# martinambrus/PitchExtractor

Hardware: AMD Instinct MI355X
Metric: mel-frames/sec training throughput (JDCNet, 24 kHz, batch=256) (higher is better)
Workload: dtype f32

## Files before the change

### pitchextractor_amd/csrc/common.h

```cpp
#pragma once
#include <hip/hip_runtime.h>
#include <stdint.h>
#include <stdlib.h>
#include <string.h>
#include "../../include/pitchextractor_hip.h"

#define PE_CHECK_HIP(expr)                              \
  do {                                                  \
    hipError_t _e = (expr);                             \
    if (_e != hipSuccess) return (int)_e;               \
  } while (0)

#define PE_LAUNCH_CHECK()                               \
  do {                                                  \
    hipError_t _e = hipGetLastError();                  \
    if (_e != hipSuccess) return (int)_e;               \
  } while (0)

static inline hipStream_t pe_stream(void* s) { return reinterpret_cast<hipStream_t>(s); }

static inline int pe_unserved(int products) {
  return products >= PE_PROD_NATIVE && products <= PE_PROD_F16 ? PE_E_UNSUPPORTED : PE_E_ARG;
}

static inline int pe_cdiv(long a, long b) { return (int)((a + b - 1) / b); }

static inline int pe_epilogue_buffer(long out_bytes) {
  static const int forced_pointer = [] {
    const char* e = getenv("PE_EPILOGUE");
    return e && strcmp(e, "pointer") == 0 ? 1 : 0;
  }();
  return !forced_pointer && out_bytes < (1L << 31);
}

typedef float f32x4 __attribute__((ext_vector_type(4)));
typedef float f32x16 __attribute__((ext_vector_type(16)));

#define PE_WAVE 64

__device__ __forceinline__ double pe_wave_strided_sum(const double* base, long stride, int n) {
  const int lane = threadIdx.x & 63;
  double s = 0.0;
  for (int z = lane; z < n; z += 64) s += base[(long)z * stride];
#pragma unroll
  for (int off = 32; off > 0; off >>= 1) s += __shfl_down(s, off, 64);
  return s;
}

static inline int pe_pick_splits(int tiles, long K, int min_k_per_split, int resident) {
  long max_s = K / min_k_per_split;
  if (max_s < 1) max_s = 1;
  if (max_s > 1024) max_s = 1024;
  int best = 1;
  double best_score = -1.0;
  for (int sp = 1; sp <= (int)max_s; ++sp) {
    const long wgs = (long)tiles * sp;
    const long waves = (wgs + resident - 1) / resident;
    const double eff = (double)wgs / (double)(waves * resident);
    const double score = eff - 0.0001 * sp + (wgs >= 2L * resident ? 0.05 : 0.0);
    if (score > best_score) { best_score = score; best = sp; }
  }
  return best;
}

__device__ __forceinline__ float4 pe_ordered_slab_sum4(const float* __restrict__ ws, long slab_stride, int splits,
                                                       long i4) {
  const float4* p = reinterpret_cast<const float4*>(ws) + i4;
  const long st4 = slab_stride >> 2;
  double sx = 0.0, sy = 0.0, sz = 0.0, sw = 0.0;
  int z = 0;
  for (; z + 8 <= splits; z += 8) {
    float4 v[8];
#pragma unroll
    for (int u = 0; u < 8; ++u) v[u] = p[(long)(z + u) * st4];
#pragma unroll
    for (int u = 0; u < 8; ++u) { sx += (double)v[u].x; sy += (double)v[u].y; sz += (double)v[u].z; sw += (double)v[u].w; }
  }
  for (; z < splits; ++z) {
    const float4 v = p[(long)z * st4];
    sx += (double)v.x; sy += (double)v.y; sz += (double)v.z; sw += (double)v.w;
  }
  return make_float4((float)sx, (float)sy, (float)sz, (float)sw);
}

__device__ __forceinline__ void philox_round(uint32_t (&c)[4], uint32_t (&k)[2]) {
  const uint32_t M0 = 0xD2511F53u, M1 = 0xCD9E8D57u;
  const uint64_t p0 = (uint64_t)M0 * c[0], p1 = (uint64_t)M1 * c[2];
  const uint32_t n0 = (uint32_t)(p1 >> 32) ^ c[1] ^ k[0];
  const uint32_t n1 = (uint32_t)p1;
  const uint32_t n2 = (uint32_t)(p0 >> 32) ^ c[3] ^ k[1];
  const uint32_t n3 = (uint32_t)p0;
  c[0] = n0; c[1] = n1; c[2] = n2; c[3] = n3;
  k[0] += 0x9E3779B9u; k[1] += 0xBB67AE85u;
}

__device__ __forceinline__ void philox4(uint64_t seed, uint64_t ctr, uint32_t (&out)[4]) {
  uint32_t c[4] = {(uint32_t)ctr, (uint32_t)(ctr >> 32), 0u, 0u};
  uint32_t k[2] = {(uint32_t)seed, (uint32_t)(seed >> 32)};
#pragma unroll
  for (int i = 0; i < 10; ++i) philox_round(c, k);
  out[0] = c[0]; out[1] = c[1]; out[2] = c[2]; out[3] = c[3];
}

__device__ __forceinline__ bool pe_dropout_keep(uint32_t word, float p) {
  return ((float)(word >> 8) * (1.0f / 16777216.0f)) >= p;
}
```

### pitchextractor_amd/csrc/gemm.hip

```cpp
#include <stdlib.h>
#include <type_traits>
#include <utility>
#include "splitk.h"


namespace {
using namespace pe;
typedef unsigned int u32x4 __attribute__((ext_vector_type(4)));

bool aligned16(const void* p) { return (reinterpret_cast<uintptr_t>(p) & 15) == 0; }

template <class TO>
struct StoreEpiT {
  TO* C;
  long ldc;
  const float* bias0;
  const float* bias1;
  int M, N, accumulate;
  __device__ __forceinline__ void operator()(int row, int col, float v) const {
    if (row < M && col < N) {
      if (bias0) v += bias0[col];
      if (bias1) v += bias1[col];
      TO* dst = C + (long)row * ldc + col;
      if (accumulate) v += ld1(dst);
// ... 124 lines not shown
        }
      }
  }
}

template <class TL, class F, class TA = typename F::TA>
int launch_nt(const RowLoaderT<TA>& al, const RowLoader& bl, const StoreEpiT<TA>& ep, int M, int N, int K,
              hipStream_t st, const unsigned* amax_a, const unsigned* amax_b) {
  constexpr int MODE = F::MODE;
  using TH = typename F::TH;
  const int tm = pe_cdiv(M, TL::BM), tn = pe_cdiv(N, TL::BN);
  const bool vec = MODE != kNative && (N & 3) == 0 && (ep.ldc & 3) == 0 &&
                   (reinterpret_cast<uintptr_t>(ep.C) & (4 * sizeof(TA) - 1)) == 0;
  if (vec) {
    if (ep.ldc >= N && pe_epilogue_buffer((long)(M + TL::BM) * ep.ldc * (long)sizeof(TA)))
      hipLaunchKernelGGL((gemm_nt_t_kernel<TL, MODE, true, TA, TH>), dim3(tm * tn), dim3(256), 0, st, al, bl, ep, K, tm,
                         tn, amax_a, amax_b);
    else
      hipLaunchKernelGGL((gemm_nt_t_kernel<TL, MODE, false, TA, TH>), dim3(tm * tn), dim3(256), 0, st, al, bl, ep, K, tm,
                         tn, amax_a, amax_b);
  }
  else
    hipLaunchKernelGGL((gemm_nt_kernel<TL, MODE, TA, TH>), dim3(tm * tn), dim3(256), 0, st, al, bl, ep, K, tm, tn, amax_a,
                       amax_b);
  PE_LAUNCH_CHECK();
  return PE_OK;
}

}

template <class F, class TA = typename F::TA>
static int gemm_nt_impl(const TA* A, long lda, const float* B, long ldb, TA* C, long ldc, int M, int N,
                        int K, const float* bias0, const float* bias1, int accumulate, void* stream,
                        const unsigned* amax_a, const unsigned* amax_b) {
  constexpr int MODE = F::MODE;
  if (!A || !B || !C || M < 0 || N < 0 || K <= 0) return PE_E_ARG;
  if (MODE == kSplit2 && (!amax_a || !amax_b)) return PE_E_ARG;
  if (M == 0 || N == 0) return PE_OK;
  if ((K & 3) || (lda & 3) || (ldb & 3) || (reinterpret_cast<uintptr_t>(A) & (4 * sizeof(TA) - 1)) || !aligned16(B))
    return PE_E_UNSUPPORTED;
  if (lda < 0 || ldb < 0 || lda >= (1L << 21) || ldb >= (1L << 21)) return PE_E_UNSUPPORTED;
  RowLoaderT<TA> al{A, lda, M, K, 0};
  RowLoader bl{B, ldb, N, K, 0};
  StoreEpiT<TA> ep{C, ldc, bias0, bias1, M, N, accumulate};
  hipStream_t st = pe_stream(stream);
  if (N <= 32) return launch_nt<Tile<128, 32, 4, 1>, F>(al, bl, ep, M, N, K, st, amax_a, amax_b);
  if (N <= 64) return launch_nt<Tile<256, 64, 4, 1>, F>(al, bl, ep, M, N, K, st, amax_a, amax_b);
  if (N % 192 == 0 && (N % 128 != 0 || MODE != kNative))
    return launch_nt<Tile<128, 192, 2, 2>, F>(al, bl, ep, M, N, K, st, amax_a, amax_b);
  return launch_nt<Tile<128, 128, 2, 2>, F>(al, bl, ep, M, N, K, st, amax_a, amax_b);
}

extern "C" int pe_gemm_nt(int products, int act16, const void* A, long lda, const float* B, long ldb, void* C, long ldc,
                          int M, int N, int K, const float* bias0, const float* bias1, int accumulate,
                          const unsigned* amax_a, const unsigned* amax_b, void* stream) {
  return with_form<kAllForms, true>(products, act16, [&](auto f) {
    using TA = typename decltype(f)::TA;
    return gemm_nt_impl<decltype(f)>(static_cast<const TA*>(A), lda, B, ldb, static_cast<TA*>(C), ldc, M, N, K, bias0,
                                     bias1, accumulate, stream, amax_a, amax_b);
  });
}

extern "C" size_t pe_gemm_tn_workspace_bytes(int M, int N, int K) {
  if (M <= 0 || N <= 0 || K <= 0) return 0;
  const int s = tn_max_splits(pe_cdiv(M, M <= 64 ? 64 : 128) * pe_cdiv(N, N <= 64 ? 64 : 128), K);
  return s > 1 ? (size_t)s * M * N * sizeof(float) : 0;
}

template <class F, class TA = typename F::TA>
static int gemm_tn_impl(const TA* A, long lda, const TA* B, long ldb, float* C, long ldc, int M, int N,
                        int K, int accumulate, float* workspace, size_t workspace_bytes, void* stream,
                        const unsigned* amax_a, const unsigned* amax_b) {
  constexpr int MODE = F::MODE;
  if (!A || !B || !C || M < 0 || N < 0 || K <= 0) return PE_E_ARG;
  if (MODE == kSplit2 && (!amax_a || !amax_b)) return PE_E_ARG;
  if (M == 0 || N == 0) return PE_OK;
  if ((M & 3) || (N & 3) || (lda & 3) || (ldb & 3) || (reinterpret_cast<uintptr_t>(A) & (4 * sizeof(TA) - 1)) ||
      (reinterpret_cast<uintptr_t>(B) & (4 * sizeof(TA) - 1)))
    return PE_E_UNSUPPORTED;
  if (lda < 0 || ldb < 0 || lda >= (1L << 24) || ldb >= (1L << 24)) return PE_E_UNSUPPORTED;
  hipStream_t st = pe_stream(stream);
  auto launch = [&](auto bm, auto bn) {
    constexpr int BM = decltype(bm)::value, BN = decltype(bn)::value;
    return launch_tn<BM, BN, F>(KRowLoader<BM, TA>{A, lda, M, 0}, KRowLoader<BN, TA>{B, ldb, N, 0}, C, ldc, M, N, K,
                                accumulate, workspace, workspace_bytes, st, amax_a, amax_b);
  };
  std::integral_constant<int, 64> t64;
  std::integral_constant<int, 128> t128;
  if (M <= 64 && N <= 64) return launch(t64, t64);
  if (M <= 64) return launch(t64, t128);
  if (N <= 64) return launch(t128, t64);
  return launch(t128, t128);
}

extern "C" int pe_gemm_tn(int products, int act16, const void* A, long lda, const void* B, long ldb, float* C, long ldc,
                          int M, int N, int K, int accumulate, float* workspace, size_t workspace_bytes,
                          const unsigned* amax_a, const unsigned* amax_b, void* stream) {
  return with_form<kAllForms, true>(products, act16, [&](auto f) {
    using TA = typename decltype(f)::TA;
    return gemm_tn_impl<decltype(f)>(static_cast<const TA*>(A), lda, static_cast<const TA*>(B), ldb, C, ldc, M, N, K,
                                     accumulate, workspace, workspace_bytes, stream, amax_a, amax_b);
  });
}
```

### pitchextractor_amd/csrc/gemm_engine.h

```cpp
#pragma once
#include <type_traits>
#include <utility>
#include "act16.h"

namespace pe {

constexpr int kBK = 32;
constexpr int kNative = 0;
constexpr int kBf16 = 1;
constexpr int kSplit = 2;
constexpr int kSplit2 = 3;
template <int MODE> constexpr int mode_terms() { return MODE == kSplit ? 3 : MODE == kSplit2 ? 2 : 1; }
constexpr int kLdsStride = kBK + 4;

template <int BM_, int BN_, int WAVES_M_, int WAVES_N_>
struct Tile {
  static constexpr int BM = BM_, BN = BN_;
  static constexpr int WAVES_M = WAVES_M_, WAVES_N = WAVES_N_;
  static constexpr int WM = BM / WAVES_M, WN = BN / WAVES_N;
  static constexpr int TM = WM / 32, TN = WN / 32;
  static constexpr int A_LOADS = BM / 32, B_LOADS = BN / 32;
  static_assert(WAVES_M * WAVES_N == 4, "4 waves per workgroup");
  static_assert(WM % 32 == 0 && WN % 32 == 0, "wave tile is a multiple of the 32x32 MFMA");
};
// ... 377 lines not shown
#pragma unroll
      for (int i = 0; i < TL::B_LOADS; ++i) rb[q][i] = bl.load(i, kt + PF);
    }
    if constexpr (PF == 2) __builtin_amdgcn_sched_barrier(0);
#pragma unroll
    for (int kk = 0; kk < kBK / 16; ++kk) {
      half8<H> fa[TL::TM][NT], fb[TL::TN][NT];
#pragma unroll
      for (int i = 0; i < TL::TM; ++i)
#pragma unroll
        for (int c = 0; c < NT; ++c)
          fa[i][c] = *reinterpret_cast<const half8<H>*>(As + c * A_IMG + swz_off(wm * TL::WM + i * 32 + r, kk * 2 + h));
#pragma unroll
      for (int j = 0; j < TL::TN; ++j)
#pragma unroll
        for (int c = 0; c < NT; ++c)
          fb[j][c] = *reinterpret_cast<const half8<H>*>(Bs + c * B_IMG + swz_off(wn * TL::WN + j * 32 + r, kk * 2 + h));
#pragma unroll
      for (int i = 0; i < TL::TM; ++i)
#pragma unroll
        for (int j = 0; j < TL::TN; ++j) acc[i][j] = mfma_terms<NT, SW>(fa[i], fb[j], acc[i][j]);
    }
    if constexpr (PF == 2) __builtin_amdgcn_sched_barrier(0);
  };
  int kt = 0;
  if constexpr (PF == 2) {
    for (; kt + 1 < nk; kt += 2) {
      tile(std::integral_constant<int, 0>{}, kt);
      tile(std::integral_constant<int, 1>{}, kt + 1);
    }
  }
  for (; kt < nk; ++kt) tile(std::integral_constant<int, 0>{}, kt);
}

template <class F, int... Q>
__device__ __forceinline__ void static_for_impl(F&& f, std::integer_sequence<int, Q...>) {
  (f(std::integral_constant<int, Q>{}), ...);
}
template <int N, class F>
__device__ __forceinline__ void static_for(F&& f) { static_for_impl(f, std::make_integer_sequence<int, N>{}); }

template <int MODE> constexpr int nt_row_floats() {
  return MODE == kSplit ? kSplitRowFloats : MODE == kSplit2 ? 2 * kBK / 2 : kLdsStride;
}

template <class TL, int MODE, bool SW = false, int PF = 1, class TH = __bf16, class AL, class BL>
__device__ __forceinline__ void nt_mainloop_mode(AL& al, BL& bl, int K, float* As, float* Bs,
                                                 f32x16 (&acc)[TL::TM][TL::TN], float sa = 1.0f, float sb = 1.0f) {
  if constexpr (MODE == kBf16) nt_mainloop_half<TL, TH>(al, bl, K, As, Bs, acc);
  else if constexpr (MODE == kSplit) nt_mainloop_split<TL, SW, 3, PF>(al, bl, K, As, Bs, acc);
  else if constexpr (MODE == kSplit2) nt_mainloop_split<TL, SW, 2, PF>(al, bl, K, As, Bs, acc, sa, sb);
  else nt_mainloop<TL>(al, bl, K, As, Bs, acc);
}

template <class TL, class FN>
__device__ __forceinline__ void for_each_acc(const f32x16 (&acc)[TL::TM][TL::TN], FN&& fn) {
  const int lane = threadIdx.x & 63, wv = threadIdx.x >> 6;
  const int wm = wv / TL::WAVES_N, wn = wv % TL::WAVES_N;
  const int r = lane & 31, h = lane >> 5;
#pragma unroll
  for (int i = 0; i < TL::TM; ++i)
#pragma unroll
    for (int j = 0; j < TL::TN; ++j)
#pragma unroll
      for (int g = 0; g < 16; ++g) {
        const int row = wm * TL::WM + i * 32 + (g & 3) + 8 * (g >> 2) + 4 * h;
        const int col = wn * TL::WN + j * 32 + r;
        fn(row, col, acc[i][j][g]);
      }
}

template <class TL>
__device__ __forceinline__ void zero_acc(f32x16 (&acc)[TL::TM][TL::TN]) {
#pragma unroll
  for (int i = 0; i < TL::TM; ++i)
#pragma unroll
    for (int j = 0; j < TL::TN; ++j)
#pragma unroll
      for (int g = 0; g < 16; ++g) acc[i][j][g] = 0.0f;
}

template <int COLS>
struct TnGeom {
  static constexpr int TPR = COLS / 4;
  static constexpr int ROWS = 256 / TPR;
  static constexpr int SLOTS = kBK / ROWS;
  static_assert(COLS == 64 || COLS == 128 || COLS == 256, "TN tile widths");
  __device__ static __forceinline__ int col4() { return (threadIdx.x % TPR) * 4; }
  __device__ static __forceinline__ int krow(int slot) { return threadIdx.x / TPR + ROWS * slot; }
};

template <int COLS, class TA = float>
struct KRowLoader {
  const TA* p;
  long ld;
  int cols;
  int col0;
  unsigned vo_ = 0, rowstep_ = 0;
  typedef typename RawQuad<TA>::type Raw;
  __device__ __forceinline__ void init(int first_col, int ) {
    col0 = first_col + TnGeom<COLS>::col4();
    vo_ = (unsigned)(((long)(threadIdx.x / TnGeom<COLS>::TPR) * ld + col0) * (long)sizeof(TA)) | (col0 < cols ? 0u : 0x80000000u);
    rowstep_ = (unsigned)(TnGeom<COLS>::ROWS * ld * (long)sizeof(TA));
  }
  __device__ __forceinline__ Raw load(int slot, int k0, int k_end) const {
    const long left = (long)k_end - k0;
    long bytes = left > 0 ? ((left - 1) * ld + cols) * (long)sizeof(TA) : 0;
    const __amdgpu_buffer_rsrc_t rs = __builtin_amdgcn_make_buffer_rsrc(
        const_cast<TA*>(p + (long)k0 * ld), 0, (unsigned)(bytes < 0x7fffffffL ? bytes : 0x7fffffffL), 0x00020000);
    return ldraw_buffer<TA>(rs, vo_ + (unsigned)slot * rowstep_, 0u);
  }
};

template <int COLS>
struct ShiftedPixelLoader {
  const float* p;
  int T, F, C, dt, df;
  int col0;
  int t_[TnGeom<COLS>::SLOTS], f_[TnGeom<COLS>::SLOTS];
  __device__ __forceinline__ void init(int first_col, int k_begin) {
    col0 = first_col + TnGeom<COLS>::col4();
#pragma unroll
    for (int i = 0; i < TnGeom<COLS>::SLOTS; ++i) {
      const int k = k_begin + TnGeom<COLS>::krow(i);
      f_[i] = k % F;
      t_[i] = (k / F) % T;
    }
  }
  __device__ __forceinline__ float4 load(int slot, int k0, int k_end) {
    const int k = k0 + TnGeom<COLS>::krow(slot);
    const int tt = t_[slot] + dt, ff = f_[slot] + df;
    float4 v = make_float4(0.f, 0.f, 0.f, 0.f);
    if (k < k_end && col0 < C && tt >= 0 && tt < T && ff >= 0 && ff < F)
      v = *reinterpret_cast<const float4*>(p + ((long)k + dt * F + df) * C + col0);
    int f = f_[slot] + kBK, t = t_[slot];
    while (f >= F) { f -= F; ++t; }
    while (t >= T) t -= T;
    f_[slot] = f; t_[slot] = t;
    return v;
  }
};

template <int COLS>
struct ShiftedTimeLoader {
  const float* p;
  long ld;
  int T, dt, cols;
  int col0;
  int t_[TnGeom<COLS>::SLOTS];
  __device__ __forceinline__ void init(int first_col, int k_begin) {
    col0 = first_col + TnGeom<COLS>::col4();
#pragma unroll
    for (int i = 0; i < TnGeom<COLS>::SLOTS; ++i) t_[i] = (k_begin + TnGeom<COLS>::krow(i)) % T;
  }
  __device__ __forceinline__ float4 load(int slot, int k0, int k_end) {
    const int k = k0 + TnGeom<COLS>::krow(slot);
    const int t = t_[slot] + dt;
    float4 v = make_float4(0.f, 0.f, 0.f, 0.f);
    if (k < k_end && col0 < cols && t >= 0 && t < T)
      v = *reinterpret_cast<const float4*>(p + ((long)k + dt) * ld + col0);
    int tn = t_[slot] + kBK;
    while (tn >= T) tn -= T;
    t_[slot] = tn;
    return v;
  }
};

template <int BM, int BN, class AL, class BL>
__device__ __forceinline__ void tn_mainloop(AL& al, BL& bl, int k_begin, int k_end, float* As, float* Bs,
                                            f32x16 (&acc)[BM / 64][BN / 64]) {
  constexpr int TM = BM / 64, TN = BN / 64;
  constexpr int SA = TnGeom<BM>::SLOTS, SB = TnGeom<BN>::SLOTS;
  const int tid = threadIdx.x, lane = tid & 63, wv = tid >> 6;
  const int wm = wv >> 1, wn = wv & 1;
  const int r = lane & 31, h = lane >> 5;
  float4 ra[SA], rb[SB];
#pragma unroll
  for (int i = 0; i < SA; ++i) ra[i] = al.load(i, k_begin, k_end);
#pragma unroll
  for (int i = 0; i < SB; ++i) rb[i] = bl.load(i, k_begin, k_end);
  const int sta = (tid / TnGeom<BM>::TPR) * BM + TnGeom<BM>::col4();
  const int stb = (tid / TnGeom<BN>::TPR) * BN + TnGeom<BN>::col4();
  const float* a_rd = As + h * BM + wm * (BM / 2) + r;
  const float* b_rd = Bs + h * BN + wn * (BN / 2) + r;
  for (int k0 = k_begin; k0 < k_end; k0 += kBK) {
    __syncthreads();
#pragma unroll
    for (int i = 0; i < SA; ++i) *reinterpret_cast<float4*>(As + sta + i * TnGeom<BM>::ROWS * BM) = ra[i];
#pragma unroll
    for (int i = 0; i < SB; ++i) *reinterpret_cast<float4*>(Bs + stb + i * TnGeom<BN>::ROWS * BN) = rb[i];
    __syncthreads();
    if (k0 + kBK < k_end) {
#pragma unroll
      for (int i = 0; i < SA; ++i) ra[i] = al.load(i, k0 + kBK, k_end);
#pragma unroll
      for (int i = 0; i < SB; ++i) rb[i] = bl.load(i, k0 + kBK, k_end);
    }
#pragma unroll
    for (int s = 0; s < kBK / 2; ++s) {
      float fa[TM], fb[TN];
#pragma unroll
      for (int i = 0; i < TM; ++i) fa[i] = a_rd[s * 2 * BM + i * 32];
#pragma unroll
      for (int j = 0; j < TN; ++j) fb[j] = b_rd[s * 2 * BN + j * 32];
#pragma unroll
      for (int i = 0; i < TM; ++i)
#pragma unroll
        for (int j = 0; j < TN; ++j) acc[i][j] = mfma32(fa[i], fb[j], acc[i][j]);
    }
  }
}

typedef short s16x4 __attribute__((ext_vector_type(4)));
template <int COLS> constexpr int tn_split_stride() { return COLS + 32; }
template <int COLS, int NT = 3> constexpr int tn_split_floats() { return NT * kBK * tn_split_stride<COLS>() / 2; }

template <class H>
__device__ __forceinline__ s16x4 lds_read_tr(const H* p) {
  return __builtin_amdgcn_ds_read_tr16_b64_v4i16(
      (__attribute__((address_space(3))) s16x4*)(reinterpret_cast<const short*>(p)));
}

template <class H>
__device__ __forceinline__ half8<H> tr_fragment(const H* p, int stride) {
  const s16x4 lo = lds_read_tr(p), hi = lds_read_tr(p + 4 * stride);
  typedef short s16x8 __attribute__((ext_vector_type(8)));
  const s16x8 v = {lo[0], lo[1], lo[2], lo[3], hi[0], hi[1], hi[2], hi[3]};
  return __builtin_bit_cast(half8<H>, v);
}

template <int COLS, int NT, class H>
__device__ __forceinline__ void tn_split_store(H* img, int off, const float4& v, float scale = 1.0f) {
  constexpr int IMG = kBK * tn_split_stride<COLS>();
  if constexpr (NT == 3) {
    const Split3 sp = split3(v);
    *reinterpret_cast<uint2*>(img + off) = sp.hi;
    *reinterpret_cast<uint2*>(img + off + IMG) = sp.mid;
    *reinterpret_cast<uint2*>(img + off + 2 * IMG) = sp.lo;
  } else if constexpr (NT == 2) {
    const Split2 sp = split2(v, scale);
    *reinterpret_cast<uint2*>(img + off) = sp.hi;
    *reinterpret_cast<uint2*>(img + off + IMG) = sp.lo;
  } else {
    *reinterpret_cast<half4<H>*>(img + off) = to_half4<H>(v);
  }
}

template <int COLS, int NT, class H>
__device__ __forceinline__ void tn_split_store(H* img, int off, const uint2& raw, float scale = 1.0f) {
  if constexpr (NT == 1) *reinterpret_cast<half4<H>*>(img + off) = to_half4<H>(raw);
  else tn_split_store<COLS, NT>(img, off, widen(raw), scale);
}

template <int BM, int BN, int NT, int PF = 1, class TH = __bf16, class AL, class BL>
__device__ __forceinline__ void tn_mainloop_split(AL& al, BL& bl, int k_begin, int k_end, float* As_f, float* Bs_f,
                                                  f32x16 (&acc)[BM / 64][BN / 64], float sa = 1.0f, float sb = 1.0f) {
  constexpr int TM = BM / 64, TN = BN / 64;
  constexpr int SA = TnGeom<BM>::SLOTS, SB = TnGeom<BN>::SLOTS;
  constexpr int STA = tn_split_stride<BM>(), STB = tn_split_stride<BN>();
  constexpr int IMGA = kBK * STA, IMGB = kBK * STB;
  using H = term_t<NT, TH>;
  H* As = reinterpret_cast<H*>(As_f);
  H* Bs = reinterpret_cast<H*>(Bs_f);
  const int tid = threadIdx.x, lane = tid & 63, wv = tid >> 6;
  const int wm = wv >> 1, wn = wv & 1;
  const int h = lane >> 5, g1 = (lane >> 4) & 1, q = (lane & 15) >> 2, p4 = (lane & 3) * 4;
  decltype(al.load(0, 0, 0)) ra[PF][SA];
  decltype(bl.load(0, 0, 0)) rb[PF][SB];
#pragma unroll
  for (int u = 0; u < PF; ++u) {
#pragma unroll
    for (int i = 0; i < SA; ++i) ra[u][i] = al.load(i, k_begin + u * kBK, k_end);
#pragma unroll
    for (int i = 0; i < SB; ++i) rb[u][i] = bl.load(i, k_begin + u * kBK, k_end);
  }
  const int sta = (tid / TnGeom<BM>::TPR) * STA + TnGeom<BM>::col4();
  const int stb = (tid / TnGeom<BN>::TPR) * STB + TnGeom<BN>::col4();
  const H* a_rd = As + (8 * h + q) * STA + wm * (BM / 2) + 16 * g1 + p4;
  const H* b_rd = Bs + (8 * h + q) * STB + wn * (BN / 2) + 16 * g1 + p4;
  auto tile = [&](auto uc, int k0) {
    constexpr int u = decltype(uc)::value;
    __syncthreads();
#pragma unroll
    for (int i = 0; i < SA; ++i) tn_split_store<BM, NT>(As, sta + i * TnGeom<BM>::ROWS * STA, ra[u][i], sa);
#pragma unroll
    for (int i = 0; i < SB; ++i) tn_split_store<BN, NT>(Bs, stb + i * TnGeom<BN>::ROWS * STB, rb[u][i], sb);
    __syncthreads();
    if (PF == 2 || k0 + kBK < k_end) {
#pragma unroll
      for (int i = 0; i < SA; ++i) ra[u][i] = al.load(i, k0 + PF * kBK, k_end);
#pragma unroll
      for (int i = 0; i < SB; ++i) rb[u][i] = bl.load(i, k0 + PF * kBK, k_end);
    }
    if constexpr (PF == 2) __builtin_amdgcn_sched_barrier(0);
#pragma unroll
    for (int kk = 0; kk < kBK / 16; ++kk) {
      half8<H> fa[TM][NT], fb[TN][NT];
#pragma unroll
      for (int i = 0; i < TM; ++i)
#pragma unroll
        for (int c = 0; c < NT; ++c) fa[i][c] = tr_fragment(a_rd + c * IMGA + kk * 16 * STA + i * 32, STA);
#pragma unroll
      for (int j = 0; j < TN; ++j)
#pragma unroll
        for (int c = 0; c < NT; ++c) fb[j][c] = tr_fragment(b_rd + c * IMGB + kk * 16 * STB + j * 32, STB);
#pragma unroll
      for (int i = 0; i < TM; ++i)
#pragma unroll
        for (int j = 0; j < TN; ++j) acc[i][j] = mfma_terms<NT>(fa[i], fb[j], acc[i][j]);
    }
    if constexpr (PF == 2) __builtin_amdgcn_sched_barrier(0);
  };
  int k0 = k_begin;
  if constexpr (PF == 2) {
    for (; k0 + kBK < k_end; k0 += 2 * kBK) {
      tile(std::integral_constant<int, 0>{}, k0);
      tile(std::integral_constant<int, 1>{}, k0 + kBK);
    }
  }
  for (; k0 < k_end; k0 += kBK) tile(std::integral_constant<int, 0>{}, k0);
}

template <int MODE, int COLS> constexpr int tn_lds_floats() {
  return MODE == kSplit ? tn_split_floats<COLS, 3>() : MODE == kSplit2 ? tn_split_floats<COLS, 2>()
       : MODE == kBf16 ? tn_split_floats<COLS, 1>() : kBK * COLS;
}

template <int MODE, int BM, int BN, int PF = 1, class TH = __bf16, class AL, class BL>
__device__ __forceinline__ void tn_mainloop_mode(AL& al, BL& bl, int k_begin, int k_end, float* As, float* Bs,
                                                 f32x16 (&acc)[BM / 64][BN / 64], float sa = 1.0f, float sb = 1.0f) {
  if constexpr (MODE == kSplit) tn_mainloop_split<BM, BN, 3, PF>(al, bl, k_begin, k_end, As, Bs, acc);
  else if constexpr (MODE == kSplit2) tn_mainloop_split<BM, BN, 2, PF>(al, bl, k_begin, k_end, As, Bs, acc, sa, sb);
  else if constexpr (MODE == kBf16) tn_mainloop_split<BM, BN, 1, PF, TH>(al, bl, k_begin, k_end, As, Bs, acc);
  else tn_mainloop<BM, BN>(al, bl, k_begin, k_end, As, Bs, acc);
}

template <class AL, class BL>
__device__ __forceinline__ void nn_mainloop_64(AL& al, BL& bl, int K, float* As, float* Bs, f32x16& acc) {
  const int tid = threadIdx.x, lane = tid & 63, wv = tid >> 6;
  const int wm = wv >> 1, wn = wv & 1;
  const int r = lane & 31, h = lane >> 5;
  const int nk = (K + kBK - 1) / kBK;
  float4 ra[2], rb[2];
  ra[0] = al.load(0, 0); ra[1] = al.load(1, 0);
  rb[0] = bl.load(0, 0, K); rb[1] = bl.load(1, 0, K);
  const int sta = (tid >> 3) * kLdsStride + (tid & 7) * 4;
  const int stb = (tid / TnGeom<64>::TPR) * 64 + TnGeom<64>::col4();
  const float* a_rd = As + (wm * 32 + r) * kLdsStride + h * 4;
  const float* b_rd = Bs + (h * 4) * 64 + wn * 32 + r;
  for (int kt = 0; kt < nk; ++kt) {
    __syncthreads();
    *reinterpret_cast<float4*>(As + sta) = ra[0];
    *reinterpret_cast<float4*>(As + sta + 32 * kLdsStride) = ra[1];
    *reinterpret_cast<float4*>(Bs + stb) = rb[0];
    *reinterpret_cast<float4*>(Bs + stb + TnGeom<64>::ROWS * 64) = rb[1];
    __syncthreads();
    if (kt + 1 < nk) {
      ra[0] = al.load(0, kt + 1); ra[1] = al.load(1, kt + 1);
      rb[0] = bl.load(0, (kt + 1) * kBK, K); rb[1] = bl.load(1, (kt + 1) * kBK, K);
    }
#pragma unroll
    for (int k8 = 0; k8 < kBK / 8; ++k8) {
      const float4 fa = *reinterpret_cast<const float4*>(a_rd + k8 * 8);
      acc = mfma32(fa.x, b_rd[(k8 * 8 + 0) * 64], acc);
      acc = mfma32(fa.y, b_rd[(k8 * 8 + 1) * 64], acc);
      acc = mfma32(fa.z, b_rd[(k8 * 8 + 2) * 64], acc);
      acc = mfma32(fa.w, b_rd[(k8 * 8 + 3) * 64], acc);
    }
  }
}

template <int BM, int BN>
__device__ __forceinline__ void tn_zero_acc(f32x16 (&acc)[BM / 64][BN / 64]) {
#pragma unroll
  for (int i = 0; i < BM / 64; ++i)
#pragma unroll
    for (int j = 0; j < BN / 64; ++j)
#pragma unroll
      for (int g = 0; g < 16; ++g) acc[i][j][g] = 0.f;
}

template <int BM, int BN, class FN>
__device__ __forceinline__ void tn_for_each_acc(const f32x16 (&acc)[BM / 64][BN / 64], FN&& fn) {
  const int lane = threadIdx.x & 63, wv = threadIdx.x >> 6;
  const int wm = wv >> 1, wn = wv & 1;
  const int r = lane & 31, h = lane >> 5;
#pragma unroll
  for (int i = 0; i < BM / 64; ++i)
#pragma unroll
    for (int j = 0; j < BN / 64; ++j)
#pragma unroll
      for (int g = 0; g < 16; ++g)
        fn(wm * (BM / 2) + i * 32 + (g & 3) + 8 * (g >> 2) + 4 * h, wn * (BN / 2) + j * 32 + r, acc[i][j][g]);
}

}
```

### pitchextractor_amd/csrc/lstm.hip

```cpp
#include "splitk.h"

namespace {
using namespace pe;

constexpr int kMaxCells = 4;

struct FwdCells {
  const float* whh[kMaxCells];
  float* gates[kMaxCells];
  float* y[kMaxCells];
  float* c[kMaxCells];
  int reverse[kMaxCells];
};

struct GateRowLoader {
  const float* p;
  int H, j0;
  __device__ __forceinline__ void init(int) {}
  __device__ __forceinline__ float4 load(int slot, int kt) const {
    const int row = slot * H + j0 + (threadIdx.x >> 3);
    const int k = kt * kBK + (threadIdx.x & 7) * 4;
    if (k < H) return *reinterpret_cast<const float4*>(p + (long)row * H + k);
    return make_float4(0.f, 0.f, 0.f, 0.f);
  }
// ... 167 lines not shown
      for (int u = 0; u < 4; ++u) { s[0] += v[u].x; s[1] += v[u].y; s[2] += v[u].z; s[3] += v[u].w; }
    }
    for (; r < r1; r += 4) {
      const float4 v = *reinterpret_cast<const float4*>(x + r * ld + c);
      s[0] += v.x; s[1] += v.y; s[2] += v.z; s[3] += v.w;
    }
  }
#pragma unroll
  for (int e = 0; e < 4; ++e) red[ry][q * 4 + e] = s[e];
  __syncthreads();
  const int cc = blockIdx.x * 256 + threadIdx.x;
  if (cc < cols)
    partial[(long)blockIdx.y * cols + cc] = (red[0][threadIdx.x] + red[1][threadIdx.x]) +
                                            (red[2][threadIdx.x] + red[3][threadIdx.x]);
}

__global__ void colsum_final_kernel(const double* __restrict__ partial, int nparts, int cols, float* out0,
                                    float* out1) {
  const int c = blockIdx.x * 4 + (threadIdx.x >> 6);
  if (c >= cols) return;
  const double s = pe_wave_strided_sum(partial + c, (long)cols, nparts);
  if ((threadIdx.x & 63) != 0) return;
  out0[c] = (float)s;
  if (out1) out1[c] = (float)s;
}

constexpr int kColsumParts = 256;

}

extern "C" int pe_lstm_fwd(int ncells, const float* const* whh, float* const* gates, float* const* y,
                           float* const* cbuf, const int* reverse, long ldy, int B, int T, int H, void* stream) {
  if (ncells < 1 || ncells > kMaxCells || !whh || !gates || !y || !cbuf || !reverse) return PE_E_ARG;
  if (B <= 0 || T <= 0 || H <= 0) return PE_E_ARG;
  if ((H % 32) != 0 || (ldy & 3)) return PE_E_UNSUPPORTED;
  FwdCells cells{};
  for (int i = 0; i < ncells; ++i) {
    if (!whh[i] || !gates[i] || !y[i] || !cbuf[i]) return PE_E_ARG;
    cells.whh[i] = whh[i]; cells.gates[i] = gates[i]; cells.y[i] = y[i]; cells.c[i] = cbuf[i];
    cells.reverse[i] = reverse[i];
  }
  dim3 grid(pe_cdiv(B, 64), H / 32, ncells);
  hipStream_t st = pe_stream(stream);
  for (int s = 0; s < T; ++s) {
    hipLaunchKernelGGL(lstm_fwd_step_kernel, grid, dim3(256), 0, st, cells, s, B, T, H, ldy);
  }
  PE_LAUNCH_CHECK();
  return PE_OK;
}

extern "C" int pe_lstm_bwd(int ncells, const float* const* whh_t, float* const* gates, const float* const* cbuf,
                           const float* const* dy, float* const* dcarry, const int* reverse, long lddy, int B,
                           int T, int H, void* stream) {
  if (ncells < 1 || ncells > kMaxCells || !whh_t || !gates || !cbuf || !dy || !dcarry || !reverse) return PE_E_ARG;
  if (B <= 0 || T <= 0 || H <= 0) return PE_E_ARG;
  if ((H % 32) != 0 || (lddy & 3)) return PE_E_UNSUPPORTED;
  BwdCells cells{};
  for (int i = 0; i < ncells; ++i) {
    if (!whh_t[i] || !gates[i] || !cbuf[i] || !dy[i] || !dcarry[i]) return PE_E_ARG;
    cells.whh_t[i] = whh_t[i]; cells.gates[i] = gates[i]; cells.c[i] = cbuf[i]; cells.dy[i] = dy[i];
    cells.dcarry[i] = dcarry[i]; cells.reverse[i] = reverse[i];
  }
  dim3 grid(pe_cdiv(B, 64), H / 32, ncells);
  hipStream_t st = pe_stream(stream);
  for (int s = 0; s < T; ++s) {
    hipLaunchKernelGGL(lstm_bwd_step_kernel, grid, dim3(256), 0, st, cells, s, B, T, H, lddy);
  }
  PE_LAUNCH_CHECK();
  return PE_OK;
}

extern "C" size_t pe_lstm_whh_grad_workspace_bytes(int B, int T, int H) {
  return (size_t)tn_max_splits(pe_cdiv(4 * H, 128) * pe_cdiv(H, 128), B * T) * 4 * H * H * sizeof(float);
}

template <class F>
static int whh_grad_impl(const float* dgates, const float* y, long ldy, float* dwhh, int B, int T, int H,
                         int reverse, float* workspace, size_t workspace_bytes, void* stream,
                         const unsigned* amax_dg, const unsigned* amax_y) {
  if (!dgates || !y || !dwhh || B <= 0 || T <= 0 || H <= 0) return PE_E_ARG;
  if (F::MODE == kSplit2 && (!amax_dg || !amax_y)) return PE_E_ARG;
  if ((H & 3) || (ldy & 3)) return PE_E_UNSUPPORTED;
  const int M = 4 * H, N = H;
  KRowLoader<128> al{dgates, (long)M, M, 0};
  ShiftedTimeLoader<128> bl;
  bl.p = y; bl.ld = ldy; bl.T = T; bl.dt = reverse ? 1 : -1; bl.cols = N; bl.col0 = 0;
  return launch_tn<128, 128, F>(al, bl, dwhh, (long)N, M, N, B * T, 0, workspace, workspace_bytes, pe_stream(stream),
                                amax_dg, amax_y);
}

extern "C" int pe_lstm_whh_grad(int products, const float* dgates, const float* y, long ldy, float* dwhh, int B, int T,
                                int H, int reverse, float* workspace, size_t workspace_bytes,
                                const unsigned* amax_dgates, const unsigned* amax_y, void* stream) {
  return with_form<kAllForms, false>(products, 0, [&](auto f) {
    return whh_grad_impl<decltype(f)>(dgates, y, ldy, dwhh, B, T, H, reverse, workspace, workspace_bytes, stream,
                                      amax_dgates, amax_y);
  });
}

extern "C" size_t pe_colsum_workspace_bytes(int cols) { return (size_t)kColsumParts * cols * sizeof(double); }

extern "C" int pe_colsum(const float* x, long rows, int cols, long ld, float* out0, float* out1, void* workspace,
                         size_t workspace_bytes, void* stream) {
  if (!x || !out0 || rows <= 0 || cols <= 0) return PE_E_ARG;
  if ((cols & 3) || (ld & 3) || (reinterpret_cast<uintptr_t>(x) & 15)) return PE_E_UNSUPPORTED;
  if (!workspace || workspace_bytes < pe_colsum_workspace_bytes(cols)) return PE_E_WORKSPACE;
  double* partial = reinterpret_cast<double*>(workspace);
  const int parts = rows < kColsumParts ? (int)rows : kColsumParts;
  hipStream_t st = pe_stream(stream);
  hipLaunchKernelGGL(colsum_partial_kernel, dim3(pe_cdiv(cols, 256), parts), dim3(256), 0, st, x, rows, cols, ld,
                     partial);
  PE_LAUNCH_CHECK();
  hipLaunchKernelGGL(colsum_final_kernel, dim3(pe_cdiv(cols, 4)), dim3(256), 0, st, partial, parts, cols, out0,
                     out1);
  PE_LAUNCH_CHECK();
  return PE_OK;
}
```

### pitchextractor_amd/csrc/splitk.h

```cpp
#pragma once
#include "forms.h"

namespace pe {

struct SplitK { int splits, kps; };

constexpr int resident_wgs(int per_cu) { return 256 * per_cu; }
constexpr int tn_resident(int mode) { return resident_wgs(mode == kSplit || mode == kSplit2 ? 2 : 3); }
constexpr int kTnMinKps = 512;

static inline SplitK splitk_plan(int tiles, int K, int min_kps, int resident) {
  const int s = pe_pick_splits(tiles, K, min_kps, resident);
  const int kps = pe_cdiv(pe_cdiv(K, s), kBK) * kBK;
  return {pe_cdiv(K, kps), kps};
}

static inline int tn_max_splits(int tiles, int K) {
  const int a = splitk_plan(tiles, K, kTnMinKps, tn_resident(kNative)).splits;
  const int b = splitk_plan(tiles, K, kTnMinKps, tn_resident(kSplit)).splits;
  return a > b ? a : b;
}

struct SplitKBlock { int m0, n0, kb, ke, split_id; };

template <int BM, int BN>
__device__ __forceinline__ SplitKBlock splitk_block(int tiles_m, int tiles_n, int K, int kps) {
  const int tiles_mn = tiles_m * tiles_n;
  const int lin = xcd_remap(blockIdx.x, gridDim.x);
  const int tile_id = lin % tiles_mn, split_id = lin / tiles_mn;
  const int m0 = (tile_id / tiles_n) * BM, n0 = (tile_id % tiles_n) * BN;
  const int kb = split_id * kps;
  const int ke = min(K, kb + kps);
  return {m0, n0, kb, ke, split_id};
}

struct RowMajorDst {
  float* C;
  long ldc;
  int M, N, accumulate;
  __host__ __device__ long elems() const { return (long)M * N; }
  __device__ __forceinline__ void operator()(long i4, const float4& s) const {
    const long idx = i4 * 4;
    const int row = (int)(idx / N), col = (int)(idx - (long)row * N);
    float* d = C + (long)row * ldc + col;
    if (accumulate) { d[0] += s.x; d[1] += s.y; d[2] += s.z; d[3] += s.w; }
    else { d[0] = s.x; d[1] = s.y; d[2] = s.z; d[3] = s.w; }
  }
};

namespace {

template <int BM, int BN, int MODE, class AL, class BL, class TH>
__global__ __launch_bounds__(256) void tn_splitk_kernel(AL al, BL bl, float* out, long ldo, long split_stride, int M,
                                                        int N, int K, int k_per_split, int tiles_n, int accumulate,
                                                        const unsigned* amax_a, const unsigned* amax_b) {
  __shared__ __attribute__((aligned(16))) float As[tn_lds_floats<MODE, BM>()];
  __shared__ __attribute__((aligned(16))) float Bs[tn_lds_floats<MODE, BN>()];
  const SplitKBlock b = splitk_block<BM, BN>((M + BM - 1) / BM, tiles_n, K, k_per_split);
  al.init(b.m0, b.kb);
  bl.init(b.n0, b.kb);
  f32x16 acc[BM / 64][BN / 64];
  tn_zero_acc<BM, BN>(acc);
  H2Scales hs{1.f, 1.f, 1.f};
  if constexpr (MODE == kSplit2) hs.load(amax_a, amax_b);
  tn_mainloop_mode<MODE, BM, BN, 1, TH>(al, bl, b.kb, b.ke, As, Bs, acc, hs.sa, hs.sb);
  float* dst = out + (long)b.split_id * split_stride;
  tn_for_each_acc<BM, BN>(acc, [&](int r, int c, float v) {
    const int row = b.m0 + r, col = b.n0 + c;
    if constexpr (MODE == kSplit2) v = hs.unscale(v);
    if (row < M && col < N) {
      float* d = dst + (long)row * ldo + col;
      if (accumulate) v += *d;
      *d = v;
    }
  });
}

template <class Dst>
__global__ void splitk_reduce_kernel(const float* ws, long split_stride, int splits, Dst dst) {
  const long i4 = (long)blockIdx.x * blockDim.x + threadIdx.x;
  if (i4 * 4 >= dst.elems()) return;
  dst(i4, pe_ordered_slab_sum4(ws, split_stride, splits, i4));
}

template <class Dst>
int launch_splitk_reduce(const float* ws, int splits, const Dst& dst, hipStream_t st) {
  const long n = dst.elems();
  hipLaunchKernelGGL(splitk_reduce_kernel<Dst>, dim3(pe_cdiv(n / 4, 256)), dim3(256), 0, st, ws, n, splits, dst);
  PE_LAUNCH_CHECK();
  return PE_OK;
}

template <int BM, int BN, class F, class AL, class BL>
int launch_tn(const AL& al, const BL& bl, float* C, long ldc, int M, int N, int K, int accumulate, float* ws,
              size_t ws_bytes, hipStream_t st, const unsigned* amax_a, const unsigned* amax_b) {
  constexpr int MODE = F::MODE;
  const int tm = pe_cdiv(M, BM), tn = pe_cdiv(N, BN);
  const SplitK p = splitk_plan(tm * tn, K, kTnMinKps, tn_resident(MODE));
  auto kernel = tn_splitk_kernel<BM, BN, MODE, AL, BL, typename F::TH>;
  if (p.splits == 1) {
    hipLaunchKernelGGL(kernel, dim3(tm * tn), dim3(256), 0, st, al, bl, C, ldc, 0L, M, N, K, p.kps, tn, accumulate,
                       amax_a, amax_b);
    PE_LAUNCH_CHECK();
    return PE_OK;
  }
  if (!ws || ws_bytes < (size_t)p.splits * M * N * sizeof(float)) return PE_E_WORKSPACE;
  hipLaunchKernelGGL(kernel, dim3(tm * tn * p.splits), dim3(256), 0, st, al, bl, ws, (long)N, (long)M * N, M, N, K,
                     p.kps, tn, 0, amax_a, amax_b);
  PE_LAUNCH_CHECK();
  return launch_splitk_reduce(ws, p.splits, RowMajorDst{C, ldc, M, N, accumulate}, st);
}

}
}
```

Before: 643,400.

## Add 192-wide TN GEMM tiles with swapped MFMA operands and buffer quad epilogue

Adds 192x192, 192x128 and 128x192 tile variants for the TN split-K GEMM and the LSTM W_hh gradient. Tiles are chosen when they pad M and N no more than 128-wide tiles would. The loaders split a 192-wide row into three 64-column chunks. Non-native modes swap the MFMA operand order so each lane holds four consecutive columns, which allows float4 buffer-store epilogues. Split planning still uses 128-tile counts, and 192 tiles request 2 blocks per CU. The trade-off is higher LDS and register pressure against better reuse and fewer tiles, and this only runs for the bf16/split forms.

```diff
diff --git a/pitchextractor_amd/csrc/common.h b/pitchextractor_amd/csrc/common.h
--- a/pitchextractor_amd/csrc/common.h
+++ b/pitchextractor_amd/csrc/common.h
@@ -31,6 +31,19 @@
     return e && strcmp(e, "pointer") == 0 ? 1 : 0;
   }();
   return !forced_pointer && out_bytes < (1L << 31);
+}
+
+static inline int pe_tn_tile_override() {
+  static const int tile = [] {
+    const char* e = getenv("PE_TN_TILE");
+    if (!e) return 0;
+    if (strcmp(e, "128") == 0) return 128128;
+    if (strcmp(e, "192") == 0 || strcmp(e, "192x192") == 0) return 192192;
+    if (strcmp(e, "128x192") == 0) return 128192;
+    if (strcmp(e, "192x128") == 0) return 192128;
+    return 0;
+  }();
+  return tile;
 }
 
 typedef float f32x4 __attribute__((ext_vector_type(4)));
diff --git a/pitchextractor_amd/csrc/gemm.hip b/pitchextractor_amd/csrc/gemm.hip
--- a/pitchextractor_amd/csrc/gemm.hip
+++ b/pitchextractor_amd/csrc/gemm.hip
@@ -230,15 +230,25 @@
   hipStream_t st = pe_stream(stream);
   auto launch = [&](auto bm, auto bn) {
     constexpr int BM = decltype(bm)::value, BN = decltype(bn)::value;
-    return launch_tn<BM, BN, F>(KRowLoader<BM, TA>{A, lda, M, 0}, KRowLoader<BN, TA>{B, ldb, N, 0}, C, ldc, M, N, K,
-                                accumulate, workspace, workspace_bytes, st, amax_a, amax_b);
+    return launch_tn<BM, BN, F, (BM < 128 ? BM : 128), (BN < 128 ? BN : 128)>(
+        KRowLoader<BM, TA>{A, lda, M, 0}, KRowLoader<BN, TA>{B, ldb, N, 0}, C, ldc, M, N, K, accumulate, workspace,
+        workspace_bytes, st, amax_a, amax_b);
   };
   std::integral_constant<int, 64> t64;
   std::integral_constant<int, 128> t128;
+  std::integral_constant<int, 192> t192;
   if (M <= 64 && N <= 64) return launch(t64, t64);
   if (M <= 64) return launch(t64, t128);
   if (N <= 64) return launch(t128, t64);
-  return launch(t128, t128);
+  const int tile = tn_tile_for(M, N, {192192, 192128, 128192});
+  int rc = kTnNarrowTile;
+  if constexpr (tn_tile_fits<MODE, 192, 192>())
+    if (tile == 192192) rc = launch(t192, t192);
+  if constexpr (tn_tile_fits<MODE, 192, 128>())
+    if (tile == 192128) rc = launch(t192, t128);
+  if constexpr (tn_tile_fits<MODE, 128, 192>())
+    if (tile == 128192) rc = launch(t128, t192);
+  return rc != kTnNarrowTile ? rc : launch(t128, t128);
 }
 
 extern "C" int pe_gemm_tn(int products, int act16, const void* A, long lda, const void* B, long ldb, float* C, long ldc,
diff --git a/pitchextractor_amd/csrc/gemm_engine.h b/pitchextractor_amd/csrc/gemm_engine.h
--- a/pitchextractor_amd/csrc/gemm_engine.h
+++ b/pitchextractor_amd/csrc/gemm_engine.h
@@ -483,12 +483,16 @@
 
 template <int COLS>
 struct TnGeom {
-  static constexpr int TPR = COLS / 4;
+  static constexpr int CHUNKS = COLS == 192 ? 3 : 1;
+  static constexpr int CW = COLS / CHUNKS;
+  static constexpr int TPR = CW / 4;
   static constexpr int ROWS = 256 / TPR;
-  static constexpr int SLOTS = kBK / ROWS;
-  static_assert(COLS == 64 || COLS == 128 || COLS == 256, "TN tile widths");
+  static constexpr int SLOTS = CHUNKS * kBK / ROWS;
+  static_assert(COLS == 64 || COLS == 128 || COLS == 192 || COLS == 256, "TN tile widths");
   __device__ static __forceinline__ int col4() { return (threadIdx.x % TPR) * 4; }
-  __device__ static __forceinline__ int krow(int slot) { return threadIdx.x / TPR + ROWS * slot; }
+  static constexpr int chunk_col(int slot) { return (slot % CHUNKS) * CW; }
+  __device__ static __forceinline__ int krow(int slot) { return threadIdx.x / TPR + ROWS * (slot / CHUNKS); }
+  static constexpr int lds_off(int slot, int stride) { return (slot / CHUNKS) * ROWS * stride + chunk_col(slot); }
 };
 
 template <int COLS, class TA = float>
@@ -497,11 +501,15 @@
   long ld;
   int cols;
   int col0;
-  unsigned vo_ = 0, rowstep_ = 0;
+  unsigned vo_[TnGeom<COLS>::CHUNKS] = {}, rowstep_ = 0;
   typedef typename RawQuad<TA>::type Raw;
   __device__ __forceinline__ void init(int first_col, int ) {
     col0 = first_col + TnGeom<COLS>::col4();
-    vo_ = (unsigned)(((long)(threadIdx.x / TnGeom<COLS>::TPR) * ld + col0) * (long)sizeof(TA)) | (col0 < cols ? 0u : 0x80000000u);
+#pragma unroll
+    for (int c = 0; c < TnGeom<COLS>::CHUNKS; ++c) {
+      const int col = col0 + TnGeom<COLS>::chunk_col(c);
+      vo_[c] = (unsigned)(((long)(threadIdx.x / TnGeom<COLS>::TPR) * ld + col) * (long)sizeof(TA)) | (col < cols ? 0u : 0x80000000u);
+    }
     rowstep_ = (unsigned)(TnGeom<COLS>::ROWS * ld * (long)sizeof(TA));
   }
   __device__ __forceinline__ Raw load(int slot, int k0, int k_end) const {
@@ -509,7 +517,7 @@
     long bytes = left > 0 ? ((left - 1) * ld + cols) * (long)sizeof(TA) : 0;
     const __amdgpu_buffer_rsrc_t rs = __builtin_amdgcn_make_buffer_rsrc(
         const_cast<TA*>(p + (long)k0 * ld), 0, (unsigned)(bytes < 0x7fffffffL ? bytes : 0x7fffffffL), 0x00020000);
-    return ldraw_buffer<TA>(rs, vo_ + (unsigned)slot * rowstep_, 0u);
+    return ldraw_buffer<TA>(rs, vo_[slot % TnGeom<COLS>::CHUNKS] + (unsigned)(slot / TnGeom<COLS>::CHUNKS) * rowstep_, 0u);
   }
 };
 
@@ -548,21 +556,26 @@
   long ld;
   int T, dt, cols;
   int col0;
-  int t_[TnGeom<COLS>::SLOTS];
+  int t_[TnGeom<COLS>::SLOTS / TnGeom<COLS>::CHUNKS];
   __device__ __forceinline__ void init(int first_col, int k_begin) {
     col0 = first_col + TnGeom<COLS>::col4();
 #pragma unroll
-    for (int i = 0; i < TnGeom<COLS>::SLOTS; ++i) t_[i] = (k_begin + TnGeom<COLS>::krow(i)) % T;
+    for (int i = 0; i < TnGeom<COLS>::SLOTS / TnGeom<COLS>::CHUNKS; ++i)
+      t_[i] = (k_begin + TnGeom<COLS>::krow(i * TnGeom<COLS>::CHUNKS)) % T;
   }
   __device__ __forceinline__ float4 load(int slot, int k0, int k_end) {
+    constexpr int CH = TnGeom<COLS>::CHUNKS;
     const int k = k0 + TnGeom<COLS>::krow(slot);
-    const int t = t_[slot] + dt;
+    const int col = col0 + TnGeom<COLS>::chunk_col(slot);
+    const int t = t_[slot / CH] + dt;
     float4 v = make_float4(0.f, 0.f, 0.f, 0.f);
-    if (k < k_end && col0 < cols && t >= 0 && t < T)
-      v = *reinterpret_cast<const float4*>(p + ((long)k + dt) * ld + col0);
-    int tn = t_[slot] + kBK;
-    while (tn >= T) tn -= T;
-    t_[slot] = tn;
+    if (k < k_end && col < cols && t >= 0 && t < T)
+      v = *reinterpret_cast<const float4*>(p + ((long)k + dt) * ld + col);
+    if (slot % CH == CH - 1) {
+      int tn = t_[slot / CH] + kBK;
+      while (tn >= T) tn -= T;
+      t_[slot / CH] = tn;
+    }
     return v;
   }
 };
@@ -587,9 +600,9 @@
   for (int k0 = k_begin; k0 < k_end; k0 += kBK) {
     __syncthreads();
 #pragma unroll
-    for (int i = 0; i < SA; ++i) *reinterpret_cast<float4*>(As + sta + i * TnGeom<BM>::ROWS * BM) = ra[i];
-#pragma unroll
-    for (int i = 0; i < SB; ++i) *reinterpret_cast<float4*>(Bs + stb + i * TnGeom<BN>::ROWS * BN) = rb[i];
+    for (int i = 0; i < SA; ++i) *reinterpret_cast<float4*>(As + sta + TnGeom<BM>::lds_off(i, BM)) = ra[i];
+#pragma unroll
+    for (int i = 0; i < SB; ++i) *reinterpret_cast<float4*>(Bs + stb + TnGeom<BN>::lds_off(i, BN)) = rb[i];
     __syncthreads();
     if (k0 + kBK < k_end) {
 #pragma unroll
@@ -653,7 +666,7 @@
   else tn_split_store<COLS, NT>(img, off, widen(raw), scale);
 }
 
-template <int BM, int BN, int NT, int PF = 1, class TH = __bf16, class AL, class BL>
+template <int BM, int BN, int NT, int PF = 1, class TH = __bf16, bool SW = false, class AL, class BL>
 __device__ __forceinline__ void tn_mainloop_split(AL& al, BL& bl, int k_begin, int k_end, float* As_f, float* Bs_f,
                                                   f32x16 (&acc)[BM / 64][BN / 64], float sa = 1.0f, float sb = 1.0f) {
   constexpr int TM = BM / 64, TN = BN / 64;
@@ -683,9 +696,9 @@
     constexpr int u = decltype(uc)::value;
     __syncthreads();
 #pragma unroll
-    for (int i = 0; i < SA; ++i) tn_split_store<BM, NT>(As, sta + i * TnGeom<BM>::ROWS * STA, ra[u][i], sa);
-#pragma unroll
-    for (int i = 0; i < SB; ++i) tn_split_store<BN, NT>(Bs, stb + i * TnGeom<BN>::ROWS * STB, rb[u][i], sb);
+    for (int i = 0; i < SA; ++i) tn_split_store<BM, NT>(As, sta + TnGeom<BM>::lds_off(i, STA), ra[u][i], sa);
+#pragma unroll
+    for (int i = 0; i < SB; ++i) tn_split_store<BN, NT>(Bs, stb + TnGeom<BN>::lds_off(i, STB), rb[u][i], sb);
     __syncthreads();
     if (PF == 2 || k0 + kBK < k_end) {
 #pragma unroll
@@ -708,7 +721,10 @@
 #pragma unroll
       for (int i = 0; i < TM; ++i)
 #pragma unroll
-        for (int j = 0; j < TN; ++j) acc[i][j] = mfma_terms<NT>(fa[i], fb[j], acc[i][j]);
+        for (int j = 0; j < TN; ++j) {
+          if constexpr (SW) acc[i][j] = mfma_terms<NT, true>(fb[j], fa[i], acc[i][j]);
+          else acc[i][j] = mfma_terms<NT>(fa[i], fb[j], acc[i][j]);
+        }
     }
     if constexpr (PF == 2) __builtin_amdgcn_sched_barrier(0);
   };
@@ -727,12 +743,13 @@
        : MODE == kBf16 ? tn_split_floats<COLS, 1>() : kBK * COLS;
 }
 
-template <int MODE, int BM, int BN, int PF = 1, class TH = __bf16, class AL, class BL>
+template <int MODE, int BM, int BN, int PF = 1, class TH = __bf16, bool SW = false, class AL, class BL>
 __device__ __forceinline__ void tn_mainloop_mode(AL& al, BL& bl, int k_begin, int k_end, float* As, float* Bs,
                                                  f32x16 (&acc)[BM / 64][BN / 64], float sa = 1.0f, float sb = 1.0f) {
-  if constexpr (MODE == kSplit) tn_mainloop_split<BM, BN, 3, PF>(al, bl, k_begin, k_end, As, Bs, acc);
-  else if constexpr (MODE == kSplit2) tn_mainloop_split<BM, BN, 2, PF>(al, bl, k_begin, k_end, As, Bs, acc, sa, sb);
-  else if constexpr (MODE == kBf16) tn_mainloop_split<BM, BN, 1, PF, TH>(al, bl, k_begin, k_end, As, Bs, acc);
+  static_assert(!SW || MODE != kNative, "the native fp32 TN loop is not swapped");
+  if constexpr (MODE == kSplit) tn_mainloop_split<BM, BN, 3, PF, __bf16, SW>(al, bl, k_begin, k_end, As, Bs, acc);
+  else if constexpr (MODE == kSplit2) tn_mainloop_split<BM, BN, 2, PF, __bf16, SW>(al, bl, k_begin, k_end, As, Bs, acc, sa, sb);
+  else if constexpr (MODE == kBf16) tn_mainloop_split<BM, BN, 1, PF, TH, SW>(al, bl, k_begin, k_end, As, Bs, acc);
   else tn_mainloop<BM, BN>(al, bl, k_begin, k_end, As, Bs, acc);
 }
 
@@ -795,4 +812,19 @@
         fn(wm * (BM / 2) + i * 32 + (g & 3) + 8 * (g >> 2) + 4 * h, wn * (BN / 2) + j * 32 + r, acc[i][j][g]);
 }
 
-}
+template <int BM, int BN, class FN>
+__device__ __forceinline__ void tn_for_each_quad(const f32x16 (&acc)[BM / 64][BN / 64], FN&& fn) {
+  const int lane = threadIdx.x & 63, wv = threadIdx.x >> 6;
+  const int wm = wv >> 1, wn = wv & 1;
+  const int r = lane & 31, h = lane >> 5;
+#pragma unroll
+  for (int i = 0; i < BM / 64; ++i)
+#pragma unroll
+    for (int j = 0; j < BN / 64; ++j)
+#pragma unroll
+      for (int q = 0; q < 4; ++q)
+        fn(wm * (BM / 2) + i * 32 + r, wn * (BN / 2) + j * 32 + 8 * q + 4 * h,
+           make_float4(acc[i][j][4 * q], acc[i][j][4 * q + 1], acc[i][j][4 * q + 2], acc[i][j][4 * q + 3]));
+}
+
+}
diff --git a/pitchextractor_amd/csrc/lstm.hip b/pitchextractor_amd/csrc/lstm.hip
--- a/pitchextractor_amd/csrc/lstm.hip
+++ b/pitchextractor_amd/csrc/lstm.hip
@@ -273,11 +273,23 @@
   if (F::MODE == kSplit2 && (!amax_dg || !amax_y)) return PE_E_ARG;
   if ((H & 3) || (ldy & 3)) return PE_E_UNSUPPORTED;
   const int M = 4 * H, N = H;
-  KRowLoader<128> al{dgates, (long)M, M, 0};
-  ShiftedTimeLoader<128> bl;
-  bl.p = y; bl.ld = ldy; bl.T = T; bl.dt = reverse ? 1 : -1; bl.cols = N; bl.col0 = 0;
-  return launch_tn<128, 128, F>(al, bl, dwhh, (long)N, M, N, B * T, 0, workspace, workspace_bytes, pe_stream(stream),
-                                amax_dg, amax_y);
+  auto launch = [&](auto bm, auto bn) {
+    constexpr int BM = decltype(bm)::value, BN = decltype(bn)::value;
+    KRowLoader<BM> al{dgates, (long)M, M, 0};
+    ShiftedTimeLoader<BN> bl;
+    bl.p = y; bl.ld = ldy; bl.T = T; bl.dt = reverse ? 1 : -1; bl.cols = N; bl.col0 = 0;
+    return launch_tn<BM, BN, F, 128, 128>(al, bl, dwhh, (long)N, M, N, B * T, 0, workspace, workspace_bytes,
+                                          pe_stream(stream), amax_dg, amax_y);
+  };
+  std::integral_constant<int, 128> t128;
+  std::integral_constant<int, 192> t192;
+  const int tile = tn_tile_for(M, N, {192192});
+  int rc = kTnNarrowTile;
+  if constexpr (tn_tile_fits<F::MODE, 192, 192>())
+    if (tile == 192192) rc = launch(t192, t192);
+  if constexpr (tn_tile_fits<F::MODE, 128, 192>())
+    if (tile == 128192) rc = launch(t128, t192);
+  return rc != kTnNarrowTile ? rc : launch(t128, t128);
 }
 
 extern "C" int pe_lstm_whh_grad(int products, const float* dgates, const float* y, long ldy, float* dwhh, int B, int T,
diff --git a/pitchextractor_amd/csrc/splitk.h b/pitchextractor_amd/csrc/splitk.h
--- a/pitchextractor_amd/csrc/splitk.h
+++ b/pitchextractor_amd/csrc/splitk.h
@@ -1,4 +1,5 @@
 #pragma once
+#include <initializer_list>
 #include "forms.h"
 
 namespace pe {
@@ -19,6 +20,20 @@
   const int a = splitk_plan(tiles, K, kTnMinKps, tn_resident(kNative)).splits;
   const int b = splitk_plan(tiles, K, kTnMinKps, tn_resident(kSplit)).splits;
   return a > b ? a : b;
+}
+
+template <int MODE, int BM, int BN> constexpr bool tn_tile_fits() {
+  return (BM <= 128 && BN <= 128) ||
+         (MODE != kNative && (tn_lds_floats<MODE, BM>() + tn_lds_floats<MODE, BN>()) * sizeof(float) <= 65536);
+}
+static inline int tn_tile_for(int M, int N, std::initializer_list<int> preferred) {
+  if (const int o = pe_tn_tile_override()) return o;
+  const long base = pe_cdiv(M, 128) * 128L * pe_cdiv(N, 128) * 128L;
+  for (const int t : preferred) {
+    const long bm = t / 1000, bn = t % 1000;
+    if (pe_cdiv(M, bm) * bm * pe_cdiv(N, bn) * bn <= base) return t;
+  }
+  return 128128;
 }
 
 struct SplitKBlock { int m0, n0, kb, ke, split_id; };
@@ -50,12 +65,17 @@
 
 namespace {
 
-template <int BM, int BN, int MODE, class AL, class BL, class TH>
-__global__ __launch_bounds__(256) void tn_splitk_kernel(AL al, BL bl, float* out, long ldo, long split_stride, int M,
-                                                        int N, int K, int k_per_split, int tiles_n, int accumulate,
-                                                        const unsigned* amax_a, const unsigned* amax_b) {
+template <int BM, int BN> constexpr int tn_min_blocks() { return BM == 192 || BN == 192 ? 2 : 1; }
+
+template <int BM, int BN, int MODE, bool BUF, class AL, class BL, class TH>
+__global__ __launch_bounds__(256, (tn_min_blocks<BM, BN>()))
+void tn_splitk_kernel(AL al, BL bl, float* out, long ldo, long split_stride, int M, int N, int K, int k_per_split,
+                      int tiles_n, int accumulate, const unsigned* amax_a, const unsigned* amax_b) {
+  constexpr bool SW = MODE != kNative;
+  static_assert(SW || !BUF, "the native fp32 loop keeps the scalar epilogue");
   __shared__ __attribute__((aligned(16))) float As[tn_lds_floats<MODE, BM>()];
   __shared__ __attribute__((aligned(16))) float Bs[tn_lds_floats<MODE, BN>()];
+  static_assert((tn_lds_floats<MODE, BM>() + tn_lds_floats<MODE, BN>()) * sizeof(float) <= 65536, "static LDS");
   const SplitKBlock b = splitk_block<BM, BN>((M + BM - 1) / BM, tiles_n, K, k_per_split);
   al.init(b.m0, b.kb);
   bl.init(b.n0, b.kb);
@@ -63,17 +83,40 @@
   tn_zero_acc<BM, BN>(acc);
   H2Scales hs{1.f, 1.f, 1.f};
   if constexpr (MODE == kSplit2) hs.load(amax_a, amax_b);
-  tn_mainloop_mode<MODE, BM, BN, 1, TH>(al, bl, b.kb, b.ke, As, Bs, acc, hs.sa, hs.sb);
+  tn_mainloop_mode<MODE, BM, BN, 1, TH, SW>(al, bl, b.kb, b.ke, As, Bs, acc, hs.sa, hs.sb);
   float* dst = out + (long)b.split_id * split_stride;
-  tn_for_each_acc<BM, BN>(acc, [&](int r, int c, float v) {
-    const int row = b.m0 + r, col = b.n0 + c;
-    if constexpr (MODE == kSplit2) v = hs.unscale(v);
+  auto element = [&](int row, int col, float v) {
     if (row < M && col < N) {
       float* d = dst + (long)row * ldo + col;
       if (accumulate) v += *d;
       *d = v;
     }
-  });
+  };
+  if constexpr (!SW) {
+    tn_for_each_acc<BM, BN>(acc, [&](int r, int c, float v) { element(b.m0 + r, b.n0 + c, v); });
+  } else {
+    auto unscale4 = [&](float4 v) {
+      if constexpr (MODE == kSplit2) {
+        v.x = hs.unscale(v.x); v.y = hs.unscale(v.y); v.z = hs.unscale(v.z); v.w = hs.unscale(v.w);
+      }
+      return v;
+    };
+    if constexpr (BUF) {
+      const unsigned rowb = (unsigned)ldo * 4u;
+      const __amdgpu_buffer_rsrc_t rs = __builtin_amdgcn_make_buffer_rsrc(
+          dst, 0, (unsigned)(((long)(M - 1) * ldo + N) * (long)sizeof(float)), 0x00020000);
+      tn_for_each_quad<BM, BN>(acc, [&](int r, int c, const float4& v) {
+        const int col = b.n0 + c;
+        st4_buffer(dst, rs, col < N ? (unsigned)(b.m0 + r) * rowb + (unsigned)col * 4u : kBufferOutside, unscale4(v));
+      });
+    } else {
+      tn_for_each_quad<BM, BN>(acc, [&](int r, int c, const float4& q) {
+        const float4 v = unscale4(q);
+        const int row = b.m0 + r, col = b.n0 + c;
+        element(row, col, v.x); element(row, col + 1, v.y); element(row, col + 2, v.z); element(row, col + 3, v.w);
+      });
+    }
+  }
 }
 
 template <class Dst>
@@ -91,22 +134,34 @@
   return PE_OK;
 }
 
-template <int BM, int BN, class F, class AL, class BL>
+constexpr int kTnNarrowTile = -1000;
+
+template <int BM, int BN, class F, int PM = BM, int PN = BN, class AL, class BL>
 int launch_tn(const AL& al, const BL& bl, float* C, long ldc, int M, int N, int K, int accumulate, float* ws,
               size_t ws_bytes, hipStream_t st, const unsigned* amax_a, const unsigned* amax_b) {
   constexpr int MODE = F::MODE;
+  constexpr bool WIDE = BM > 128 || BN > 128;
+  static_assert(!WIDE || MODE != kNative, "the native fp32 loop has no 192-wide tile");
   const int tm = pe_cdiv(M, BM), tn = pe_cdiv(N, BN);
-  const SplitK p = splitk_plan(tm * tn, K, kTnMinKps, tn_resident(MODE));
-  auto kernel = tn_splitk_kernel<BM, BN, MODE, AL, BL, typename F::TH>;
-  if (p.splits == 1) {
-    hipLaunchKernelGGL(kernel, dim3(tm * tn), dim3(256), 0, st, al, bl, C, ldc, 0L, M, N, K, p.kps, tn, accumulate,
-                       amax_a, amax_b);
+  const SplitK p = splitk_plan(pe_cdiv(M, PM) * pe_cdiv(N, PN), K, kTnMinKps, tn_resident(MODE));
+  auto buffer = tn_splitk_kernel<BM, BN, MODE, MODE != kNative, AL, BL, typename F::TH>;
+  auto pointer = tn_splitk_kernel<BM, BN, MODE, WIDE, AL, BL, typename F::TH>;
+  auto quads = [&](const float* out, long ldo) {
+    return MODE != kNative && (N & 3) == 0 && (ldo & 3) == 0 && ldo >= N &&
+           (reinterpret_cast<uintptr_t>(out) & 15) == 0 && pe_epilogue_buffer((long)(M + BM) * ldo * (long)sizeof(float));
+  };
+  const bool direct = p.splits == 1;
+  const bool buf = direct ? !accumulate && quads(C, ldc) : quads(ws, N);
+  if (WIDE && !buf) return kTnNarrowTile;
+  if (direct) {
+    hipLaunchKernelGGL(buf ? buffer : pointer, dim3(tm * tn), dim3(256), 0, st, al, bl, C, ldc, 0L, M, N, K, p.kps, tn,
+                       accumulate, amax_a, amax_b);
     PE_LAUNCH_CHECK();
     return PE_OK;
   }
   if (!ws || ws_bytes < (size_t)p.splits * M * N * sizeof(float)) return PE_E_WORKSPACE;
-  hipLaunchKernelGGL(kernel, dim3(tm * tn * p.splits), dim3(256), 0, st, al, bl, ws, (long)N, (long)M * N, M, N, K,
-                     p.kps, tn, 0, amax_a, amax_b);
+  hipLaunchKernelGGL(buf ? buffer : pointer, dim3(tm * tn * p.splits), dim3(256), 0, st, al, bl, ws, (long)N,
+                     (long)M * N, M, N, K, p.kps, tn, 0, amax_a, amax_b);
   PE_LAUNCH_CHECK();
   return launch_splitk_reduce(ws, p.splits, RowMajorDst{C, ldc, M, N, accumulate}, st);
 }
```

Measured after the change: 650,300 (median of 6 runs). 1.01x the previous value.
